# AlexandreRouma/qdsp

Hardware: AMD Instinct MI355X
Metric: Msamples/s complex IQ through 256-tap FIR+decimate chain, 1/2/4/8 GPU (higher is better)
Workload: dtype f32; 1 GPU; 256-tap complex FIR (real taps), synthetic IQ resident in HBM (BASELINE configs[1]); ntaps=256, decim=1, halo_samples=0, partition=single stream

## Files before the change

qdsp_amd/csrc/fft_fir.hip:

```cpp
#include "fft_fir.hip.h"
#ifndef QDSP_HIP_DIAG
#define QDSP_HIP_DIAG 0
#endif
#include "cfft.hip.h"
#include "cpk.hip.h"
#include "ldsdma.hip.h"

namespace qk {

typedef float f4v __attribute__((ext_vector_type(4)));

__host__ __device__ constexpr int pos1(int e) { return (e >> 1) + 136 * (e & 1); }

template <int DEC, bool ROT, bool REAL = false>
__global__ __launch_bounds__(kFftNT, (DEC == 1 || !ROT) ? 4 : 3) void fir_fft_kernel(const FftArgs a) {
    __shared__ __attribute__((aligned(16))) float2 lds[kFftLdsElems + 16 * 17];
    __shared__ double2 s_pb[2];
    float2* tbl = lds + kFftLdsElems;
    const int t_lane = threadIdx.x, t = t_lane;
    const int H = a.H;
    const int te_lane = (t & ~63) | ((t & 31) << 1) | ((t >> 5) & 1);
    const int te = te_lane;
    constexpr int NS = 16 / DEC;
    constexpr int NACT = 256 / DEC;

    if ((int)blockIdx.x == a.nwg) {
        if constexpr (REAL) {
            const float* inr = reinterpret_cast<const float*>(a.in);
            const float* hr = reinterpret_cast<const float*>(a.hist);
            float* hn = reinterpret_cast<float*>(a.hist_next);
            for (int i = t; i < H; i += kFftNT) {
                const long long g = a.count - H + i;
                hn[i] = g < 0 ? hr[g + H] : inr[g];
            }
            return;
        }
        for (int i = t; i < H; i += kFftNT) {
            const long long g = a.count - H + i;
            float2 v;
            if (g < 0) {
                v = a.hist_keep[g + H];
                if (ROT && a.hist_raw_next) a.hist_raw_next[i] = a.hist[g + H];
            } else {
                v = a.in[g];
                if (ROT) {
                    const double2 p = fx_phasor(a.phase_in0 + (unsigned long long)g * a.dphase);
                    const float gain = fmaf((float)(int)(g & 511), a.gm1, 1.0f);
                    if (a.hist_raw_next) a.hist_raw_next[i] = make_float2(v.x * gain, v.y * gain);
                    v = cmulc<false>(v, make_float2((float)p.x * gain, (float)p.y * gain));
                }
            }
            a.hist_next[i] = v;
        }
        return;
    }

    float2 ta[16], hf[16];
#pragma unroll
    for (int k = 0; k < 16; k++) {
        hf[k] = a.Hf[t * 16 + k];
        if (DEC == 1) ta[k] = a.TA[te * 16 + k];
    }
    const int e0 = ((t / NS) * 16 + (t % NS) * DEC) & 255;
    tbl[(t >> 4) * 17 + (t & 15)] = a.TB[t];

    float2 pl = make_float2(1.0f, 0.0f);
    if (ROT) {
        const double2 p = fx_phasor((unsigned long long)(DEC == 1 ? te : e0) * a.dphase);
        pl = make_float2((float)p.x, (float)p.y);
        if (t == 0) s_pb[0] = fx_phasor(a.phase0 + (unsigned long long)((long long)blockIdx.x * a.L - a.seg_shift) * a.dphase);
    }
    int seg_parity = 0;

    for (int b = blockIdx.x; b < a.nblocks; b += a.nwg) {
        int t_seg = t_lane;
        if constexpr (DEC == 1 ? (ROT || REAL) : !ROT) asm volatile("" : "+v"(t_seg));
        const int t = t_seg, hi = t >> 4, lo = t & 15;
        const int te = (t & ~63) | ((t & 31) << 1) | ((t >> 5) & 1), half = (t >> 5) & 1, pte = pos1(te);
        const float2* tb = tbl + lo * 17;
        const long long seg0 = (long long)(REAL ? 2 * b : b) * a.L - a.seg_shift;
        const long long segB = seg0 + a.L;
        const bool interior = seg0 >= 0 && (REAL ? segB : seg0) + kFftN <= a.count;
        float2 v[16];
        if constexpr (REAL) {
            const float* __restrict__ inr = reinterpret_cast<const float*>(a.in);
            const float* __restrict__ hr = reinterpret_cast<const float*>(a.hist);
            if (interior && a.vec) {
                const float2* __restrict__ pa = reinterpret_cast<const float2*>(inr + seg0 + (te & ~1)) + half * 8 * 128;
                const float2* __restrict__ pb = reinterpret_cast<const float2*>(inr + segB + (te & ~1)) + half * 8 * 128;
#pragma unroll
                for (int r = 0; r < 8; r++) {
                    const float2 qa = pa[r * 128], qb = pb[r * 128];
                    const auto sa = __builtin_amdgcn_permlane32_swap(__float_as_uint(qa.x), __float_as_uint(qa.y), false, false);
                    const auto sb = __builtin_amdgcn_permlane32_swap(__float_as_uint(qb.x), __float_as_uint(qb.y), false, false);
// ... 35 lines not shown
                const long long g = seg0 + n2 * 256 + te;
                float2 x = make_float2(0.0f, 0.0f);
                if (g < 0) { if (g + H >= 0) x = a.hist[g + H]; }
                else if (g < a.count) x = a.in[g];
                v[n2] = x;
            }
        }
        float2 q = make_float2(1.0f, 0.0f);
        if (ROT) {
            if (a.gm1 != 0.0f) {
                const int gb = (int)((seg0 + te) & 511);
                const float g0 = fmaf((float)gb, a.gm1, 1.0f), g1 = fmaf((float)(gb ^ 256), a.gm1, 1.0f);
                const bool nohist = seg0 >= 0;
#pragma unroll
                for (int n2 = 0; n2 < 16; n2++) {
                    const float gg = (n2 & 1) ? g1 : g0;
                    if (nohist || seg0 + n2 * 256 + te >= 0) v[n2] = make_float2(v[n2].x * gg, v[n2].y * gg);
                }
            }
        }
        auto make_q = [&]() {
            if (!ROT) return;
            const double2 pbv = s_pb[seg_parity];
            q = cmulc<false>(make_float2((float)pbv.x, (float)pbv.y), pl);
            if (t == 0) s_pb[seg_parity ^ 1] = dcmul(pbv, a.rot_step);
            seg_parity ^= 1;
        };
        auto rot_out = [&](int n2, float2 y) {
            if (!ROT) return y;
            return cmulc<false>(y, (n2 == 0) ? q : cmulc<false>(q, a.wtab[n2]));
        };
        fft16<false>(v);
        if constexpr (DEC > 1) {
            const float2* tap = a.TA + te * 16;
            asm volatile("" : "+v"(tap) : "v"(v[0].x));
#pragma unroll
            for (int k = 1; k < 16; k++) ta[k] = tap[k];
        }
        __syncthreads();
#pragma unroll
        for (int k = 0; k < 16; k++) lds[k * kFftRow1 + pte] = (k == 0) ? v[rev16(0)] : cmulc<false>(v[rev16(k)], ta[k]);
        __syncthreads();
#pragma unroll
        for (int j = 0; j < 16; j++) v[j] = lds[hi * kFftRow1 + pos1(j * 16 + lo)];
        fft16<false>(v);
        __syncthreads();
#pragma unroll
        for (int k = 0; k < 16; k++)
            lds[(hi * 16 + k) * kFftRow2 + lo] = (k == 0) ? v[rev16(0)] : cmulc<false>(v[rev16(k)], tb[k]);
        __syncthreads();
#pragma unroll
        for (int j = 0; j < 16; j++) v[j] = lds[t * kFftRow2 + j];
        fft16<false>(v);
        float2 y[16];
#pragma unroll
        for (int k = 0; k < 16; k++) y[k] = cmulc<false>(v[rev16(k)], hf[k]);
        fft16<true>(y);
        __syncthreads();
        if constexpr (DEC == 1) {
#pragma unroll
            for (int j = 0; j < 16; j++)
                lds[t * kFftRow2 + j] = (j == 0) ? y[rev16(0)] : cmulc<true>(y[rev16(j)], tb[j]);
            __syncthreads();
#pragma unroll
            for (int j = 0; j < 16; j++) v[j] = lds[(hi * 16 + j) * kFftRow2 + lo];
            fft16<true>(v);
            __syncthreads();
#pragma unroll
            for (int j = 0; j < 16; j++) lds[hi * kFftRow1 + pos1(j * 16 + lo)] = v[rev16(j)];
            __syncthreads();
// ... 73 lines not shown
                        o4[r * 128] = make_float4(__uint_as_float(sx[0]), __uint_as_float(sy[0]), __uint_as_float(sx[1]), __uint_as_float(sy[1]));
                }
            } else if (interior) {
#pragma unroll
                for (int n2 = 0; n2 < 16; n2++)
                    if (n2 * 256 + te >= a.ov) a.out[o0 + n2 * 256] = v[rev16(n2)];
            } else {
#pragma unroll
                for (int n2 = 0; n2 < 16; n2++) {
                    const long long n = o0 + n2 * 256;
                    if (n2 * 256 + te >= a.ov && n < a.nout) a.out[n] = v[rev16(n2)];
                }
            }
        } else {
#pragma unroll
            for (int s = 0; s < NS; s++) {
                const int n0 = s * DEC;
                lds[(hi * NS + s) * kFftRow2 + lo] = (n0 == 0) ? y[rev16(0)] : cmulc<true>(y[rev16(n0)], tb[n0]);
            }
            __syncthreads();
            if (t < NACT) {
#pragma unroll
                for (int j = 0; j < 16; j++) v[j] = lds[t * kFftRow2 + j];
                fft16<true>(v);
            }
            __syncthreads();
            if (t < NACT) {
                const int k0 = t / NS, s = t % NS;
#pragma unroll
                for (int j = 0; j < 16; j++) lds[(j * NS + s) * kFftRow2 + k0] = v[rev16(j)];
            }
            __syncthreads();
            if (t < NACT) {
                const float2* ta2 = a.TA + e0 * 16;
                asm volatile("" : "+v"(ta2) : "v"(v[0].x));
#pragma unroll
                for (int k = 0; k < 16; k++) {
                    const float2 e = lds[t * kFftRow2 + k];
                    v[k] = (k == 0) ? e : cmulc<true>(e, ta2[k]);
                }
                fft16<true>(v);
                make_q();
                const long long nb = ((long long)b * a.L - a.ov) / DEC;
                float2* __restrict__ seg_out = a.out + nb;
                const long long left = a.nout - nb;
                const int end_out = left < kFftN ? (int)left : kFftN;
#pragma unroll
                for (int n2 = 0; n2 < 16; n2++) {
                    const int i = n2 * 256 + e0;
                    if (i >= a.ov && i / DEC < end_out) seg_out[i / DEC] = rot_out(n2, v[rev16(n2)]);
                }
            }
        }
    }
}

#define QK_LDS_BARRIER() asm volatile("s_waitcnt lgkmcnt(0)\n\ts_barrier" ::: "memory")

__global__ __launch_bounds__(kFftNT, 4) void fir_fft_dma_kernel(const FftArgs a) {
    __shared__ __attribute__((aligned(16))) float2 lds[kFftLdsElems + 16 * 17];
    float2* tbl = lds + kFftLdsElems;
    const int t = threadIdx.x;
    const int hi = t >> 4, lo = t & 15;
    const int H = a.H;
    const int half = (t >> 4) & 1;
    const int te = (t & ~31) | ((t & 15) << 1) | half;

    if ((int)blockIdx.x == a.nwg) {
        for (int i = t; i < H; i += kFftNT) {
            const long long g = a.count - H + i;
            a.hist_next[i] = g < 0 ? a.hist_keep[g + H] : a.in[g];
        }
        return;
    }
    float2 ta[16], hf[16];
#pragma unroll
    for (int k = 0; k < 16; k++) {
        hf[k] = a.Hf[t * 16 + k];
        ta[k] = a.TA[te * 16 + k];
    }
    tbl[(t >> 4) * 17 + (t & 15)] = a.TB[t];
    const float2* tb = tbl + lo * 17;
    {
        float touch = 0.0f;
#pragma unroll
        for (int k = 0; k < 16; k++) touch += hf[k].x + hf[k].y + (k ? ta[k].x + ta[k].y : 0.0f);
        asm volatile("" ::"v"(touch));
    }
    __syncthreads();

    const int wcol = __builtin_amdgcn_readfirstlane(t & ~63);
    const unsigned lds_cols = __builtin_amdgcn_readfirstlane((unsigned)(uintptr_t)lds) + (unsigned)wcol * 8u;
    const unsigned voff = (unsigned)(t & 31) * 16u;
    auto seg_start = [&](int b) { return (long long)b * a.L - a.seg_shift; };
    auto is_interior = [&](int b) {
        const long long s0 = seg_start(b);
        return b < a.nblocks && s0 >= 0 && s0 + kFftN <= a.count;
    };
    auto request = [&](int b) {
        const float2* src = a.in + seg_start(b) + wcol;
        if ((t & 32) == 0) {
#pragma unroll
            for (int n2 = 0; n2 < 16; n2++) dma16_to_lds(src + n2 * 256, voff, lds_cols + (unsigned)(n2 * kFftRow1) * 8u);
        }
    };

    int b = blockIdx.x;
    bool landed_in_lds = false, eight_younger = false;
    if (b < a.nblocks && is_interior(b)) {
        request(b);
        landed_in_lds = true;
    }
    for (; b < a.nblocks; b += a.nwg) {
        const long long seg0 = seg_start(b);
        float2 v[16];
        if (landed_in_lds) {
            if (eight_younger) asm volatile("s_waitcnt vmcnt(8)" ::: "memory");
            else asm volatile("s_waitcnt vmcnt(0)" ::: "memory");
        } else {
            const int first_in = seg0 < 0 ? (int)-seg0 : 0;
            const int end_in = a.count - seg0 < kFftN ? (int)(a.count - seg0) : kFftN;
            const float2* __restrict__ seg_in = a.in + seg0;
            const float2* __restrict__ seg_hist = a.hist + (H - first_in);
            int tev = te;
            asm volatile("" : "+v"(tev));
#pragma unroll
            for (int n2 = 0; n2 < 16; n2++) {
                const int i = n2 * 256 + tev;
                float2 x = make_float2(0.0f, 0.0f);
                if (i < first_in) { if (i - first_in + H >= 0) x = seg_hist[i]; }
                else if (i < end_in) x = seg_in[i];
                lds[n2 * kFftRow1 + te] = x;
            }
        }
#pragma unroll
        for (int n2 = 0; n2 < 16; n2++) v[n2] = lds[n2 * kFftRow1 + te];
        fft16<false>(v);
#pragma unroll
        for (int k = 0; k < 16; k++) lds[k * kFftRow1 + te] = (k == 0) ? v[rev16(0)] : cmulc<false>(v[rev16(k)], ta[k]);
        QK_LDS_BARRIER();
#pragma unroll
        for (int j = 0; j < 16; j++) v[j] = lds[hi * kFftRow1 + j * 16 + lo];
        fft16<false>(v);
        QK_LDS_BARRIER();
#pragma unroll
        for (int k = 0; k < 16; k++)
            lds[(hi * 16 + k) * kFftRow2 + lo] = (k == 0) ? v[rev16(0)] : cmulc<false>(v[rev16(k)], tb[k]);
        QK_LDS_BARRIER();
#pragma unroll
        for (int j = 0; j < 16; j++) v[j] = lds[t * kFftRow2 + j];
        fft16<false>(v);
        float2 y[16];
#pragma unroll
        for (int k = 0; k < 16; k++) y[k] = cmulc<false>(v[rev16(k)], hf[k]);
        fft16<true>(y);
        QK_LDS_BARRIER();
#pragma unroll
        for (int j = 0; j < 16; j++)
            lds[t * kFftRow2 + j] = (j == 0) ? y[rev16(0)] : cmulc<true>(y[rev16(j)], tb[j]);
        QK_LDS_BARRIER();
#pragma unroll
        for (int j = 0; j < 16; j++) v[j] = lds[(hi * 16 + j) * kFftRow2 + lo];
        fft16<true>(v);
        QK_LDS_BARRIER();
#pragma unroll
        for (int j = 0; j < 16; j++) lds[hi * kFftRow1 + j * 16 + lo] = v[rev16(j)];
        QK_LDS_BARRIER();
        float2 e[16];
#pragma unroll
        for (int k = 0; k < 16; k++) e[k] = lds[k * kFftRow1 + te];
        const int nb = b + a.nwg;
        landed_in_lds = is_interior(nb);
        if (landed_in_lds) {
            asm volatile("s_waitcnt lgkmcnt(0)" ::: "memory");
            request(nb);
        }
#pragma unroll
        for (int k = 0; k < 16; k++) v[k] = (k == 0) ? e[k] : cmulc<true>(e[k], ta[k]);
        fft16<true>(v);
        eight_younger = false;
        if (seg0 >= 0 && seg0 + kFftN <= a.nout) {
            f4v* __restrict__ o4 = reinterpret_cast<f4v*>(a.out + seg0);
            int pair = (te >> 1) + half * 8 * 128;
            asm volatile("" : "+v"(pair));
#pragma unroll
            for (int r = 0; r < 8; r++) {
                const float2 lo_row = v[rev16(r)], hi_row = v[rev16(8 + r)];
                const auto sx = __builtin_amdgcn_permlane16_swap(__float_as_uint(lo_row.x), __float_as_uint(hi_row.x), false, false);
                const auto sy = __builtin_amdgcn_permlane16_swap(__float_as_uint(lo_row.y), __float_as_uint(hi_row.y), false, false);
                if ((half * 8 + r) * 256 + (te & ~1) >= a.ov)
                    o4[pair + r * 128] = (f4v){__uint_as_float(sx[0]), __uint_as_float(sy[0]), __uint_as_float(sx[1]), __uint_as_float(sy[1])};
            }
            eight_younger = true;
        } else {
            const int first_out = seg0 < 0 ? (int)-seg0 : 0;
            const int from = a.ov > first_out ? a.ov : first_out;
            const int end_out = a.nout - seg0 < kFftN ? (int)(a.nout - seg0) : kFftN;
            float2* __restrict__ seg_out = a.out + seg0;
            int tev = te;
            asm volatile("" : "+v"(tev));
#pragma unroll
            for (int n2 = 0; n2 < 16; n2++) {
                const int i = n2 * 256 + tev;
                if (i >= from && i < end_out) seg_out[i] = v[rev16(n2)];
            }
        }
    }
    asm volatile("s_waitcnt vmcnt(0)" ::: "memory");
}

template <bool CONJ, int ABL> __device__ __forceinline__ v2f abl_cmul(v2f a, v2f b) {
    if (ABL & 1) return a;
    return pk_cmul2<CONJ>(a, b);
}

template <bool STAMPS, int ABL = 0>
__global__ __launch_bounds__(kFftNT, 4) void fir_fft_dmapk_kernel(const FftArgs a) {
    __shared__ __attribute__((aligned(16))) v2f lds[kFftLdsElems + 16 * 17];
    v2f* tbl = lds + kFftLdsElems;
    const int t = threadIdx.x;
    const int hi = t >> 4, lo = t & 15;
    const int H = a.H;
    const int half = (t >> 4) & 1;
    const int te = (t & ~31) | ((t & 15) << 1) | half;

    if ((int)blockIdx.x == a.nwg) {
        for (int i = t; i < H; i += kFftNT) {
            const long long g = a.count - H + i;
            a.hist_next[i] = g < 0 ? a.hist_keep[g + H] : a.in[g];
        }
        return;
    }
    v2f ta[16], hf[16];
#pragma unroll
    for (int k = 0; k < 16; k++) {
        hf[k] = reinterpret_cast<const v2f*>(a.Hf)[t * 16 + k];
        ta[k] = reinterpret_cast<const v2f*>(a.TA)[te * 16 + k];
    }
    tbl[(t >> 4) * 17 + (t & 15)] = reinterpret_cast<const v2f*>(a.TB)[t];
    const v2f* tb = tbl + lo * 17;
    {
        float touch = 0.0f;
#pragma unroll
        for (int k = 0; k < 16; k++) touch += hf[k].x + hf[k].y + (k ? ta[k].x + ta[k].y : 0.0f);
        asm volatile("" ::"v"(touch));
    }
    __syncthreads();

    const int wcol = __builtin_amdgcn_readfirstlane(t & ~63);
    const unsigned lds_cols = __builtin_amdgcn_readfirstlane((unsigned)(uintptr_t)lds) + (unsigned)wcol * 8u;
    const unsigned voff = (unsigned)(t & 31) * 16u;
    auto seg_start = [&](int b) { return (long long)b * a.L - a.seg_shift; };
    auto is_interior = [&](int b) {
        const long long s0 = seg_start(b);
        return b < a.nblocks && s0 >= 0 && s0 + kFftN <= a.count;
    };
    auto request = [&](int b) {
        const float2* src = a.in + seg_start(b) + wcol;
        if ((t & 32) == 0 && !(ABL & 4)) {
            if (a.nt & 1) {
#pragma unroll
                for (int n2 = 0; n2 < 16; n2++) {
                    if (n2 == 0 || n2 == 15) dma16_to_lds(src + n2 * 256, voff, lds_cols + (unsigned)(n2 * kFftRow1) * 8u);
                    else dma16_to_lds_nt(src + n2 * 256, voff, lds_cols + (unsigned)(n2 * kFftRow1) * 8u);
                }
            } else {
#pragma unroll
                for (int n2 = 0; n2 < 16; n2++) dma16_to_lds(src + n2 * 256, voff, lds_cols + (unsigned)(n2 * kFftRow1) * 8u);
            }
        }
    };

    unsigned acc[16] = {0, 0, 0, 0, 0, 0, 0, 0, 0, 0, 0, 0, 0, 0, 0, 0};
    unsigned long long tick = 0;
    if constexpr (STAMPS) tick = __builtin_amdgcn_s_memtime();
#define QK_STAMP(i)                                                          \
    if constexpr (STAMPS) {                                                  \
        const unsigned long long now_ = __builtin_amdgcn_s_memtime();        \
        acc[i] += (unsigned)(now_ - tick);                                   \
        tick = now_;                                                         \
    }
    int b = blockIdx.x;
    bool landed_in_lds = false, eight_younger = false;
    if (b < a.nblocks && is_interior(b)) {
        request(b);
        landed_in_lds = true;
    }
    for (; b < a.nblocks; b += a.nwg) {
        const long long seg0 = seg_start(b);
        v2f v[16];
        QK_STAMP(15)
        if (landed_in_lds) {
            if (eight_younger) asm volatile("s_waitcnt vmcnt(8)" ::: "memory");
            else asm volatile("s_waitcnt vmcnt(0)" ::: "memory");
            QK_STAMP(0)
        } else {
            const int first_in = seg0 < 0 ? (int)-seg0 : 0;
            const int end_in = a.count - seg0 < kFftN ? (int)(a.count - seg0) : kFftN;
            const float2* __restrict__ seg_in = a.in + seg0;
            const float2* __restrict__ seg_hist = a.hist + (H - first_in);
            int tev = te;
            asm volatile("" : "+v"(tev));
#pragma unroll
            for (int n2 = 0; n2 < 16; n2++) {
                const int i = n2 * 256 + tev;
                float2 x = make_float2(0.0f, 0.0f);
                if (i < first_in) { if (i - first_in + H >= 0) x = seg_hist[i]; }
                else if (i < end_in) x = seg_in[i];
                lds[n2 * kFftRow1 + te] = mk2(x.x, x.y);
            }
        }
#pragma unroll
        for (int n2 = 0; n2 < 16; n2++) v[n2] = lds[n2 * kFftRow1 + te];
        if (!(ABL & 1)) pk_fft16<false>(v);
#pragma unroll
        for (int k = 0; k < 16; k++) lds[k * kFftRow1 + te] = (k == 0) ? v[rev16(0)] : abl_cmul<false, ABL>(v[rev16(k)], ta[k]);
        QK_STAMP(1)
        QK_LDS_BARRIER();
        QK_STAMP(2)
#pragma unroll
        for (int j = 0; j < 16; j++) v[j] = lds[hi * kFftRow1 + j * 16 + lo];
// ... 7 lines not shown
        QK_STAMP(5)
        QK_LDS_BARRIER();
        QK_STAMP(6)
#pragma unroll
        for (int j = 0; j < 16; j++) v[j] = lds[t * kFftRow2 + j];
        if (!(ABL & 1)) pk_fft16<false>(v);
        v2f y[16];
#pragma unroll
        for (int k = 0; k < 16; k++) y[k] = abl_cmul<false, ABL>(v[rev16(k)], hf[k]);
        if (!(ABL & 1)) pk_fft16<true>(y);
        QK_STAMP(7)
        QK_LDS_BARRIER();
        QK_STAMP(8)
#pragma unroll
        for (int j = 0; j < 16; j++)
            lds[t * kFftRow2 + j] = (j == 0) ? y[rev16(0)] : abl_cmul<true, ABL>(y[rev16(j)], tb[j]);
        QK_STAMP(9)
        QK_LDS_BARRIER();
        QK_STAMP(10)
#pragma unroll
        for (int j = 0; j < 16; j++) v[j] = lds[(hi * 16 + j) * kFftRow2 + lo];
        if (!(ABL & 1)) pk_fft16<true>(v);
        QK_STAMP(11)
        QK_LDS_BARRIER();
        QK_STAMP(12)
#pragma unroll
        for (int j = 0; j < 16; j++) lds[hi * kFftRow1 + j * 16 + lo] = v[rev16(j)];
        QK_STAMP(13)
        QK_LDS_BARRIER();
        QK_STAMP(14)
        v2f e[16];
#pragma unroll
        for (int k = 0; k < 16; k++) e[k] = lds[k * kFftRow1 + te];
        const int nb = b + a.nwg;
        landed_in_lds = is_interior(nb);
        if (landed_in_lds) {
            asm volatile("s_waitcnt lgkmcnt(0)" ::: "memory");
            request(nb);
        }
#pragma unroll
        for (int k = 0; k < 16; k++) v[k] = (k == 0) ? e[k] : abl_cmul<true, ABL>(e[k], ta[k]);
        if (!(ABL & 1)) pk_fft16<true>(v);
        eight_younger = false;
        if (seg0 >= 0 && seg0 + kFftN <= a.nout) {
            f4v* __restrict__ o4 = reinterpret_cast<f4v*>(a.out + seg0);
            int pair = (te >> 1) + half * 8 * 128;
            asm volatile("" : "+v"(pair));
            const bool nts = (a.nt & 2) != 0;
#pragma unroll
            for (int r = 0; r < 8; r++) {
                const v2f lo_row = v[rev16(r)], hi_row = v[rev16(8 + r)];
                const auto sx = __builtin_amdgcn_permlane16_swap(__float_as_uint(lo_row.x), __float_as_uint(hi_row.x), false, false);
                const auto sy = __builtin_amdgcn_permlane16_swap(__float_as_uint(lo_row.y), __float_as_uint(hi_row.y), false, false);
                if ((half * 8 + r) * 256 + (te & ~1) >= a.ov) {
                    const f4v o = {__uint_as_float(sx[0]), __uint_as_float(sy[0]), __uint_as_float(sx[1]), __uint_as_float(sy[1])};
                    if (ABL & 2) { if (o.x == 1.2345e30f) o4[pair + r * 128] = o; }
                    else if (nts) __builtin_nontemporal_store(o, o4 + pair + r * 128);
                    else o4[pair + r * 128] = o;
                }
            }
            eight_younger = true;
        } else {
            const int first_out = seg0 < 0 ? (int)-seg0 : 0;
            const int from = a.ov > first_out ? a.ov : first_out;
            const int end_out = a.nout - seg0 < kFftN ? (int)(a.nout - seg0) : kFftN;
            v2f* __restrict__ seg_out = reinterpret_cast<v2f*>(a.out) + seg0;
            int tev = te;
            asm volatile("" : "+v"(tev));
#pragma unroll
            for (int n2 = 0; n2 < 16; n2++) {
                const int i = n2 * 256 + tev;
                if (i >= from && i < end_out) seg_out[i] = v[rev16(n2)];
            }
        }
    }
    asm volatile("s_waitcnt vmcnt(0)" ::: "memory");
    if constexpr (STAMPS) {
        if (t == 0) {
#pragma unroll
            for (int q = 0; q < 16; q++) a.stamps[(long long)blockIdx.x * 16 + q] = acc[q];
        }
    }
#undef QK_STAMP
}

template <int DEC, bool ROT>
__global__ __launch_bounds__(kFftNT, 2) void fir_fft_dec_kernel(const FftArgs a) {
    __shared__ __attribute__((aligned(16))) float2 lds[2 * kFftLdsElems + 16 * 17];
    float2* stage = lds + kFftLdsElems;
    float2* tbl = lds + 2 * kFftLdsElems;
    const int t = threadIdx.x;
    const int hi = t >> 4, lo = t & 15;
    const int H = a.H;
    constexpr int NS = 16 / DEC;
    constexpr int NACT = 256 / DEC;

    if ((int)blockIdx.x == a.nwg) {
        for (int i = t; i < H; i += kFftNT) {
            const long long g = a.count - H + i;
            float2 v;
            if (g < 0) {
                v = a.hist_keep[g + H];
                if (ROT && a.hist_raw_next) a.hist_raw_next[i] = a.hist[g + H];
            } else {
                v = a.in[g];
                if (ROT) {
                    const double2 p = fx_phasor(a.phase_in0 + (unsigned long long)g * a.dphase);
                    const float gain = fmaf((float)(int)(g & 511), a.gm1, 1.0f);
                    if (a.hist_raw_next) a.hist_raw_next[i] = make_float2(v.x * gain, v.y * gain);
                    v = cmulc<false>(v, make_float2((float)p.x * gain, (float)p.y * gain));
                }
            }
            a.hist_next[i] = v;
        }
        return;
    }

    float2 ta[16], hf[16];
    const int wbb = t / NACT, wr = t % NACT;
    const int e0 = (wr / NS) * 16 + (wr % NS) * DEC;
#pragma unroll
    for (int k = 0; k < 16; k++) {
        hf[k] = a.Hf[t * 16 + k];
        ta[k] = a.TA[t * 16 + k];
    }
    tbl[(t >> 4) * 17 + (t & 15)] = a.TB[t];
    const float2* tb = tbl + lo * 17;

    float2 pl = make_float2(1.0f, 0.0f);
    if (ROT) {
        const double2 p = fx_phasor((unsigned long long)e0 * a.dphase);
        pl = make_float2((float)p.x, (float)p.y);
    }

    auto load_segment = [&](int b, float2 (&v)[16]) {
        const long long seg0 = (long long)b * a.L - a.seg_shift;
        if (b < a.nblocks && seg0 >= 0 && seg0 + kFftN <= a.count) {
            const float2* __restrict__ p = a.in + seg0 + t;
#pragma unroll
            for (int n2 = 0; n2 < 16; n2++) v[n2] = p[n2 * 256];
        } else {
#pragma unroll
            for (int n2 = 0; n2 < 16; n2++) {
                const long long g = seg0 + n2 * 256 + t;
                float2 x = make_float2(0.0f, 0.0f);
                if (b < a.nblocks) {
                    if (g < 0) { if (g + H >= 0) x = a.hist[g + H]; }
                    else if (g < a.count) x = a.in[g];
                }
                v[n2] = x;
            }
        }
    };

    const int ngroups = (a.nblocks + DEC - 1) / DEC;
    double2 pbg = make_double2(1.0, 0.0);
    if (ROT) pbg = fx_phasor(a.phase0 + (unsigned long long)((long long)((int)blockIdx.x * DEC + wbb) * a.L - a.seg_shift) * a.dphase);
// ... 46 lines not shown
            for (int r = 0; r < NS; r++) {
                gsum[r] = y[r];
#pragma unroll
                for (int k = r + NS; k < 16; k += NS) gsum[r] = cadd(gsum[r], y[k]);
            }
            if constexpr (NS == 4) fft4<true>(gsum[0], gsum[1], gsum[2], gsum[3]);
            if constexpr (NS == 2) {
                const float2 e = gsum[0], o = gsum[1];
                gsum[0] = cadd(e, o);
                gsum[1] = csub(e, o);
            }
#pragma unroll
            for (int s = 0; s < NS; s++) {
                const int n0 = s * DEC;
                stage[(bb * NACT + hi * NS + s) * kFftRow2 + lo] = (n0 == 0) ? gsum[0] : cmulc<true>(gsum[s], tb[n0]);
            }
            if (bb + 1 < DEC) {
#pragma unroll
                for (int n2 = 0; n2 < 16; n2++) v[n2] = vn[n2];
            }
        }
        __syncthreads();
#pragma unroll
        for (int j = 0; j < 16; j++) v[j] = stage[t * kFftRow2 + j];
        fft16<true>(v);
        {
            const int ubb = t / NACT, ur = t % NACT;
            const int k0 = ur / NS, s = ur % NS;
#pragma unroll
            for (int j = 0; j < 16; j++) lds[(ubb * NACT + j * NS + s) * kFftRow2 + k0] = v[rev16(j)];
        }
        __syncthreads();
        {
            const float2* ta2 = a.TA + e0 * 16;
            asm volatile("" : "+v"(ta2) : "v"(v[0].x));
#pragma unroll
            for (int k = 0; k < 16; k++) {
                const float2 e = lds[t * kFftRow2 + k];
                v[k] = (k == 0) ? e : cmulc<true>(e, ta2[k]);
            }
        }
        fft16<true>(v);
        const int b = b0 + wbb;
        const long long nb = ((long long)b * a.L - a.ov) / DEC;
#pragma unroll
        for (int n2 = 0; n2 < 16; n2++) {
            const int i = n2 * 256 + e0;
            const long long n = nb + i / DEC;
            float2 y = v[rev16(n2)];
            if (ROT) y = cmulc<false>(y, (n2 == 0) ? q : cmulc<false>(q, a.wtab[n2]));
            if (b < a.nblocks && i >= a.ov && n < a.nout) a.out[n] = y;
        }
    }
}

int launch_fir_fft(const FftArgs& a, int grid, hipStream_t stream) {
#define QK_FFT(dec, rot) hipLaunchKernelGGL((fir_fft_dec_kernel<dec, rot>), dim3(grid), dim3(kFftNT), 0, stream, a)
    const bool r = a.rot != 0;
    switch (a.dec) {
        case 1:
#if QDSP_HIP_DIAG
            if (a.dma == 2 && a.abl == 1) hipLaunchKernelGGL((fir_fft_dmapk_kernel<false, 1>), dim3(grid), dim3(kFftNT), 0, stream, a);
            else if (a.dma == 2 && a.abl == 2) hipLaunchKernelGGL((fir_fft_dmapk_kernel<false, 2>), dim3(grid), dim3(kFftNT), 0, stream, a);
            else if (a.dma == 2 && a.abl == 4) hipLaunchKernelGGL((fir_fft_dmapk_kernel<false, 4>), dim3(grid), dim3(kFftNT), 0, stream, a);
            else if (a.dma == 2 && a.abl == 6) hipLaunchKernelGGL((fir_fft_dmapk_kernel<false, 6>), dim3(grid), dim3(kFftNT), 0, stream, a);
            else if (a.dma == 2 && a.abl == 7) hipLaunchKernelGGL((fir_fft_dmapk_kernel<false, 7>), dim3(grid), dim3(kFftNT), 0, stream, a);
            else if (a.dma == 2 && a.stamps) hipLaunchKernelGGL(fir_fft_dmapk_kernel<true>, dim3(grid), dim3(kFftNT), 0, stream, a);
            else
#endif
            if (a.dma == 2) hipLaunchKernelGGL(fir_fft_dmapk_kernel<false>, dim3(grid), dim3(kFftNT), 0, stream, a);
            else if (a.dma) hipLaunchKernelGGL(fir_fft_dma_kernel, dim3(grid), dim3(kFftNT), 0, stream, a);
            else if (a.real2) hipLaunchKernelGGL((fir_fft_kernel<1, false, true>), dim3(grid), dim3(kFftNT), 0, stream, a);
// ... 21 lines not shown
```

qdsp_amd/csrc/fft_fir.hip.h:

```cpp
#pragma once
#include <hip/hip_runtime.h>
#include "kconst.h"

namespace qk {

constexpr int kFftNT = 256;
constexpr int kFftRow1 = 272;
constexpr int kFftRow2 = 17;
constexpr int kFftLdsElems = 16 * kFftRow1;

struct FftArgs {
    const float2* in;
    float2* out;
    const float2* hist;
    float2* hist_raw_next;
    const float2* hist_keep;
    float2* hist_next;
    const float2* Hf;
    const float2* TA;
    const float2* TB;
    long long count;
    long long nout;
    int H;
    int dec;
    int decm;
    unsigned decm_inv;
    int strided;
    int rot;
    int ov;
    int seg_shift;
    int L;
    int nblocks;
    int nwg;
    int vec;
    int grouped;
    int m_shift;
    int abl;
    unsigned* stamps;
    int nt;
    int dma;
    int real2;
    unsigned long long phase_in0;
    unsigned long long phase0;
    unsigned long long dphase;
    double2 rot_step;
    float2 wtab[16];
    float gm1;
};

constexpr int kFft1kN = 1024;
constexpr int kFft1kPitch = 84;
int launch_fir_fft1k(const FftArgs& a, hipStream_t stream);

int launch_fir_fft(const FftArgs& a, int grid, hipStream_t stream);

}
```

qdsp_amd/csrc/knobs.h:

```cpp
#pragma once
#include <atomic>

namespace qk {

#define QDSP_HIP_KNOBS(X) \
    X(ANY_SMALL_CALL_TILES) \
    X(CHAN_ABL) \
    X(CHAN_MAX_WG) X(CHAN_NO_ST4) X(DECIM_SETTING) X(FFT1K_MAX_COUNT) X(FFT_ABL) X(FFT_DMA) \
    X(FFT_MIN_TAPS_DECIM) X(FFT_MIN_TAPS_REAL) \
    X(FFT_MIN_TAPS_SMALL) X(FFT_NT) X(FFT_PRUNE2_MAX_COUNT) X(FFT_WG_PER_CU) X(FIR_LAT_MAX_WORK) X(FIR_MODE) X(FIR_PICK) X(FORCE_ANY) \
    X(LEVEL_ROW_TILES) \
    X(MF_BATCH_MIN_WORK) X(MF_DEPTH) X(MF_MIN_COUNT) X(MF_MIN_DECIM) \
    X(MF_TASK_MAX) X(NO_CHAN_BATCH) X(NO_DECIM_TABLE) X(NO_FFT1K) X(NO_FFT1K_REAL) X(NO_FIR_LAT) X(NO_FIR_TABLE) X(NO_LM) \
    X(NO_LM_SMALL_CALL_RULE) X(NO_MF) X(NO_MF_BATCH) X(NO_PFB) X(NO_RM) X(NO_RM_EXT) X(NO_SPLIT_UPLOAD) \
    X(NO_WIN) X(NT) X(PFB_MIN_COUNT) X(PFB_WG_PER_CU) X(R) X(RM_MIN_COUNT) X(RM_MIN_INTERP) \
    X(RM_WAVES_PER_SIMD) X(WIN_MAX_TAPS) X(WIN_R) 
enum Knob {
#define X(n) K_##n,
    QDSP_HIP_KNOBS(X)
#undef X
    K_COUNT
};

struct Knobs {
    int val[K_COUNT];
    unsigned char set[K_COUNT];
    unsigned long long fft_stamps;
};

const Knobs* knobs_snapshot();
void knobs_reload();

inline int knob(Knob k, int dflt) {
    const Knobs* s = knobs_snapshot();
    return s->set[k] ? s->val[k] : dflt;
}

}
```

qdsp_amd/csrc/qdsp_hip.hip:

```cpp
#include "engine.hip.h"

namespace qh {

Engine* as_engine(void* h, Kind k) {
    Engine* e = static_cast<Engine*>(h);
    if (!e || e->magic != kMagic || e->kind != k) return nullptr;
    return e;
}

long double turns_of(float re, float im) {
    const long double two_pi = 6.283185307179586476925286766559005768L;
    long double t = atan2l((long double)im, (long double)re) / two_pi;
    t -= floorl(t);
    return t;
}
unsigned long long fx_of_turns(long double t) {
    t -= floorl(t);
    long double s = ldexpl(t, 64);
    if (s >= 18446744073709551615.0L) return 0ULL;
    return (unsigned long long)s;
}
void unit_of_fx(unsigned long long ph, long double mult, double* c, double* s) {
    const long double two_pi = 6.283185307179586476925286766559005768L;
    long double t = ldexpl((long double)ph, -64) * mult;
// ... 534 lines not shown
}

void reversed_taps(const Engine* e, std::vector<long double>& gr, std::vector<long double>& gi) {
    const long double two_pi = 6.283185307179586476925286766559005768L;
    const int N = e->ntaps;
    for (int j = 0; j < N; j++) {
        const long double h = (long double)e->taps_host[N - 1 - j];
        long double c = 1.0L, sn = 0.0L;
        if (e->rotate) {
            const long double tt = ldexpl((long double)e->dphase, -64) * (long double)(N - 1 - j);
            c = cosl(two_pi * (tt - floorl(tt)));
            sn = sinl(two_pi * (tt - floorl(tt)));
        }
        gr[j] = h * c;
        gi[j] = h * sn;
    }
}

int fft_prepare(Engine* e) {
    const unsigned long long key_dphase = e->rotate ? e->dphase : 0;
    if (e->fft_ntaps == e->ntaps && e->fft_tw_ready && e->fft_dphase == key_dphase) return 0;
    constexpr int F = qk::kFftN;
    const long double two_pi = 6.283185307179586476925286766559005768L;
    std::vector<long double> cs, sn;
    if (!e->fft_tw_ready) {
        cs.resize(F);
        sn.resize(F);
        for (int i = 0; i < F; i++) {
            cs[i] = cosl(two_pi * (long double)i / F);
            sn[i] = sinl(two_pi * (long double)i / F);
        }
    }
    const int N = e->ntaps;
    std::vector<float2> Hp(F), TA(256 * 16), TB(16 * 16);
    std::vector<long double> gr(N), gi(N);
    reversed_taps(e, gr, gi);
    std::vector<double> sre, sim;
    host_spectrum(gr, gi, F, sre, sim);
    for (int k = 0; k < F; k++) {
        const int k0 = k & 15, k1 = (k >> 4) & 15, k2 = k >> 8;
        Hp[(k0 * 16 + k1) * 16 + k2] = make_float2((float)(sre[k] / F), (float)(sim[k] / F));
    }
    if (!e->fft_tw_ready) {
        for (int t = 0; t < 256; t++)
            for (int k = 0; k < 16; k++) TA[t * 16 + k] = make_float2((float)cs[(t * k) % F], (float)(-sn[(t * k) % F]));
        for (int lo = 0; lo < 16; lo++)
            for (int k = 0; k < 16; k++) TB[lo * 16 + k] = make_float2((float)cs[(16 * lo * k) % F], (float)(-sn[(16 * lo * k) % F]));
        if (!e->d_fft_H) HIPCHK(hipMalloc(&e->d_fft_H, sizeof(float2) * F));
        if (!e->d_fft_TA) HIPCHK(hipMalloc(&e->d_fft_TA, sizeof(float2) * 256 * 16));
        if (!e->d_fft_TB) HIPCHK(hipMalloc(&e->d_fft_TB, sizeof(float2) * 16 * 16));
        HIPCHK(hipMemcpy(e->d_fft_TA, TA.data(), sizeof(float2) * TA.size(), hipMemcpyHostToDevice));
        HIPCHK(hipMemcpy(e->d_fft_TB, TB.data(), sizeof(float2) * TB.size(), hipMemcpyHostToDevice));
        e->fft_tw_ready = true;
    }
    HIPCHK(hipDeviceSynchronize());
    HIPCHK(hipMemcpy(e->d_fft_H, Hp.data(), sizeof(float2) * F, hipMemcpyHostToDevice));
    e->fft_ntaps = N;
    e->fft_dphase = key_dphase;
    return 0;
}

int fft1k_prepare(Engine* e) {
    const unsigned long long key_dphase = e->rotate ? e->dphase : 0;
    if (e->f1k_ntaps == e->ntaps && e->f1k_tw_ready && e->f1k_dphase == key_dphase) return 0;
    constexpr int F = qk::kFft1kN;
    const long double two_pi = 6.283185307179586476925286766559005768L;
    std::vector<long double> cs, sn;
    if (!e->f1k_tw_ready) {
        cs.resize(F);
        sn.resize(F);
        for (int i = 0; i < F; i++) {
            cs[i] = cosl(two_pi * (long double)i / F);
            sn[i] = sinl(two_pi * (long double)i / F);
        }
    }
    const int N = e->ntaps;
    std::vector<long double> gr(N), gi(N);
    reversed_taps(e, gr, gi);
    std::vector<float2> Hp(F), T(64 * 16 + 4 * 16);
    std::vector<double> sre, sim;
    host_spectrum(gr, gi, F, sre, sim);
    for (int k = 0; k < F; k++) {
        const double re = sre[k], im = sim[k];
        const int ka = k & 15, kb1 = (k >> 4) & 15, kb0 = k >> 8;
        Hp[(4 * (kb1 & 3) + kb0) * 64 + ((ka << 2) | (kb1 >> 2))] = make_float2((float)(re / F), (float)(im / F));
    }
    if (!e->f1k_tw_ready) {
        for (int l = 0; l < 64; l++)
            for (int k = 0; k < 16; k++) T[k * 64 + l] = make_float2((float)cs[(l * k) % F], (float)(-sn[(l * k) % F]));
// ... 251 lines not shown
        unit_of_fx(a.phase0 - (unsigned long long)(8 * (a.Q - 1) + 1) * a.dphase, 1.0L, &a.pb_base.x, &a.pb_base.y);
        for (int k = 0; k < 12; k++) unit_of_fx_c(e->dphase, 8.0L * (long double)a.Lo * (long double)(1 << k), &a.seg_pow[k].x, &a.seg_pow[k].y);
        for (int b1 = 0; b1 < 8; b1++) {
            double c, sn;
            unit_of_fx_c(e->dphase, (long double)(512 * b1), &c, &sn);
            a.wtab[b1] = make_float2((float)c, (float)sn);
        }
    }
    rc = qk::launch_pfb_dec(a, s);
    if (rc) return rc;
    e->raw_valid = e->rotate && e->H > 0;
    e->last.name = a.real ? (a.PH == 2 ? "pfb_dec4_real_kernel" : "pfb_dec8_real_kernel") : a.PH == 2 ? "pfb_dec4_kernel" : "pfb_dec8_kernel";
    e->last.grid = nwg + 1;
    e->last.block = qk::kPfbNT * a.PH;
    e->last.lds = (int)((qk::kPfbTableElems + (a.PH - 1) * qk::kPfbG1Elems + wpw * 64 * qk::kPfbRow + (a.PH - 1) * wpw * 64 * 9) * sizeof(float2));
    return 0;
}

int launch_fft(Engine* e, const void* d_in, int64_t count, int64_t nout, void* d_out, hipStream_t s) {
    int rc = fft_prepare(e);
    if (rc) return rc;
    qk::FftArgs a;
    memset(&a, 0, sizeof(a));
    a.in = static_cast<const float2*>(d_in);
    a.out = static_cast<float2*>(d_out);
    a.hist = reinterpret_cast<const float2*>(e->d_hist[e->cur]);
    a.hist_keep = a.hist;
    a.hist_next = reinterpret_cast<float2*>(e->d_hist[e->cur ^ 1]);
    rc = raw_history(e, s, &a.hist, &a.hist_raw_next);
    if (rc) return rc;
    a.Hf = e->d_fft_H;
    a.TA = e->d_fft_TA;
    a.TB = e->d_fft_TB;
    a.count = count;
    a.nout = nout;
    a.H = e->H;
    a.dec = fft_dec(desc_of(e));
    if (a.dec == 2 && e->ch == 2) {
        const int lim = qk::knob(qk::K_FFT_PRUNE2_MAX_COUNT, -1);
        if (count >= (lim >= 0 ? (int64_t)lim : (int64_t)(e->rotate ? 1 << 25 : 1 << 24))) a.dec = 1;
    }
    a.rot = e->rotate ? 1 : 0;
    a.decm = 1;
    if (a.dec == 1 && e->kind != KIND_FIR) {
        a.decm = e->M;
        a.decm_inv = (e->M >= 2 && (unsigned long long)(e->M + 4096) * (unsigned long long)e->M < (1ULL << 32)) ? (unsigned)((1ULL << 32) / (unsigned)e->M) + 1u : 0u;
        a.strided = 1;
        a.ov = (e->ntaps - 1 + 1) & ~1;
        a.seg_shift = a.ov + 2;
        a.L = qk::kFftN - a.ov;
        a.nblocks = (int)((count + 2 + a.L - 1) / a.L);
        a.vec = (((uintptr_t)d_in) & 15) == 0;
    } else if (a.dec == 1) {
        a.ov = (e->ntaps - 1 + 1) & ~1;
        a.vec = ((((uintptr_t)d_in) | ((uintptr_t)d_out)) & 15) == 0;
        a.seg_shift = a.ov;
        a.L = qk::kFftN - a.ov;
        a.nblocks = (int)((count + a.L - 1) / a.L);
    } else {
        a.ov = ((e->ntaps - 1 + a.dec - 1) / a.dec) * a.dec;
        a.seg_shift = a.ov + 1;
        a.L = qk::kFftN - a.ov;
        const int per_block = a.L / a.dec;
        a.nblocks = (int)((nout + per_block - 1) / per_block);
    }
    if (e->ch == 1) {
        a.real2 = 1;
        a.vec = ((((uintptr_t)d_in) | ((uintptr_t)d_out)) & 7) == 0;
        a.nblocks = (a.nblocks + 1) / 2;
    }
    a.nt = qk::knob(qk::K_FFT_NT, 0);
    a.abl = qk::knob(qk::K_FFT_ABL, 0);
    a.stamps = reinterpret_cast<unsigned*>(qk::knobs_snapshot()->fft_stamps);
    a.dma = (a.dec == 1 && !a.strided && !a.rot && e->ch == 2 && a.vec && a.ov <= 2048) ? qk::knob(qk::K_FFT_DMA, 1) : 0;
    const bool grouped = a.dec >= 4 && (a.nblocks + a.dec - 1) / a.dec >= 1024;
    a.grouped = grouped ? 1 : 0;
    const int per_cu = qk::knob(qk::K_FFT_WG_PER_CU, grouped ? 4 : 16);
    const int units = grouped ? (a.nblocks + a.dec - 1) / a.dec : a.nblocks;
    int nwg = 256 * per_cu;
    if (nwg > units) nwg = units;
    a.nwg = nwg;
    if (a.rot) {
        a.phase_in0 = e->phase;
        a.phase0 = e->phase - (unsigned long long)(e->ntaps - 1) * e->dphase;
        a.dphase = e->dphase;
        a.gm1 = e->volk_gain ? e->gm1 : 0.0f;
        const long double step_mult = (long double)nwg * (long double)a.L * (long double)(grouped ? a.dec : 1);
        if (!e->rot_step_ok || e->rot_step_dphase != e->dphase || e->rot_step_mult != step_mult) {
            unit_of_fx_c(e->dphase, step_mult, &e->rot_step_val.x, &e->rot_step_val.y);
            e->rot_step_dphase = e->dphase;
            e->rot_step_mult = step_mult;
            e->rot_step_ok = true;
        }
        a.rot_step = e->rot_step_val;
        if (!e->wtab4k_ok || e->wtab4k_dphase != e->dphase) {
            for (int n2 = 0; n2 < 16; n2++) {
                double c, sn;
                unit_of_fx_c(e->dphase, (long double)(256 * n2), &c, &sn);
                e->wtab4k[n2] = make_float2((float)c, (float)sn);
            }
            e->wtab4k_dphase = e->dphase;
            e->wtab4k_ok = true;
        }
        memcpy(a.wtab, e->wtab4k, sizeof(a.wtab));
    }
    rc = qk::launch_fir_fft(a, nwg + 1, s);
    if (rc) return rc;
    e->raw_valid = e->rotate && e->H > 0;
    e->last.name = a.dma == 2 ? "fir_fft_dmapk_kernel" : a.dma ? "fir_fft_dma_kernel" : "fir_fft_kernel";
    e->last.grid = nwg + 1;
    e->last.block = qk::kFftNT;
    e->last.lds = (int)(((grouped ? 2 : 1) * qk::kFftLdsElems + 16 * 17) * sizeof(float2));
    return 0;
// ... 761 lines not shown
```

Measured before the change: 309,400 Msamples/s.

## Taper FFT-FIR DMA block schedule and transpose twiddle tables for coalesced loads

Adds transposed copies of the filter spectrum and twiddle tables so per-thread table loads read consecutive addresses across lanes, selected by a new knob that is on by default. In the DMA kernels, the grid-strided block loop becomes a tapered schedule: a set of long-running workgroups handles the first several rounds, and the remaining blocks are split into shrinking tiers spread over extra workgroups to reduce tail imbalance. It also adds realtime and hardware-register stamps in the diagnostic path. In exchange it doubles table memory, and the DMA path now uses a different workgroups-per-CU default (4 instead of 16) when computing slots, which changes how many workgroups are resident.

Measured after the change: 317,200 Msamples/s (median of 6 runs). 2.5% higher.

```diff
diff --git a/qdsp_amd/csrc/fft_fir.hip b/qdsp_amd/csrc/fft_fir.hip
--- a/qdsp_amd/csrc/fft_fir.hip
+++ b/qdsp_amd/csrc/fft_fir.hip
@@ -11,6 +11,15 @@
 typedef float f4v __attribute__((ext_vector_type(4)));
 
 __host__ __device__ constexpr int pos1(int e) { return (e >> 1) + 136 * (e & 1); }
+
+struct FftTbl {
+    const float2 *hf, *ta;
+    int ks;
+    unsigned ls;
+};
+__device__ __forceinline__ FftTbl fft_tbl(const FftArgs& a) {
+    return a.tbl ? FftTbl{a.HfT, a.TAT, 256, 1u} : FftTbl{a.Hf, a.TA, 1, 16u};
+}
 
 template <int DEC, bool ROT, bool REAL = false>
 __global__ __launch_bounds__(kFftNT, (DEC == 1 || !ROT) ? 4 : 3) void fir_fft_kernel(const FftArgs a) {
@@ -55,11 +64,12 @@
         return;
     }
 
+    const FftTbl T = fft_tbl(a);
     float2 ta[16], hf[16];
 #pragma unroll
     for (int k = 0; k < 16; k++) {
-        hf[k] = a.Hf[t * 16 + k];
-        if (DEC == 1) ta[k] = a.TA[te * 16 + k];
+        hf[k] = (T.hf + k * T.ks)[(unsigned)t * T.ls];
+        if (DEC == 1) ta[k] = (T.ta + k * T.ks)[(unsigned)te * T.ls];
     }
     const int e0 = ((t / NS) * 16 + (t % NS) * DEC) & 255;
     tbl[(t >> 4) * 17 + (t & 15)] = a.TB[t];
@@ -161,10 +171,11 @@
         };
         fft16<false>(v);
         if constexpr (DEC > 1) {
-            const float2* tap = a.TA + te * 16;
-            asm volatile("" : "+v"(tap) : "v"(v[0].x));
-#pragma unroll
-            for (int k = 1; k < 16; k++) ta[k] = tap[k];
+            unsigned tap = (unsigned)te * T.ls;
+            int ks = T.ks;
+            asm volatile("" : "+v"(tap), "+s"(ks) : "v"(v[0].x));
+#pragma unroll
+            for (int k = 1; k < 16; k++) ta[k] = (T.ta + k * ks)[tap];
         }
         __syncthreads();
 #pragma unroll
@@ -304,12 +315,13 @@
             }
             __syncthreads();
             if (t < NACT) {
-                const float2* ta2 = a.TA + e0 * 16;
-                asm volatile("" : "+v"(ta2) : "v"(v[0].x));
+                unsigned ta2 = (unsigned)e0 * T.ls;
+                int ks = T.ks;
+                asm volatile("" : "+v"(ta2), "+s"(ks) : "v"(v[0].x));
 #pragma unroll
                 for (int k = 0; k < 16; k++) {
                     const float2 e = lds[t * kFftRow2 + k];
-                    v[k] = (k == 0) ? e : cmulc<true>(e, ta2[k]);
+                    v[k] = (k == 0) ? e : cmulc<true>(e, (T.ta + k * ks)[ta2]);
                 }
                 fft16<true>(v);
                 make_q();
@@ -328,6 +340,28 @@
 }
 
 #define QK_LDS_BARRIER() asm volatile("s_waitcnt lgkmcnt(0)\n\ts_barrier" ::: "memory")
+
+__device__ __forceinline__ void fft_run_of(const FftArgs& a, int w, int& b, int& step, int& left) {
+    if (w < a.n_long) {
+        b = w;
+        step = a.n_long;
+        left = (a.nblocks - w + a.n_long - 1) / a.n_long;
+        if (left > a.rounds) left = a.rounds;
+        return;
+    }
+    int seg = a.rounds * a.n_long, wg = a.n_long, rem = a.nblocks - seg, len = 1;
+    while (rem > 0) {
+        int cnt;
+        len = fft_taper_tier(rem, a.n_long, cnt);
+        if (w < wg + cnt) break;
+        wg += cnt;
+        seg += cnt * len;
+        rem -= cnt * len;
+    }
+    b = seg + (w - wg) * len;
+    step = 1;
+    left = a.nblocks - b < len ? a.nblocks - b : len;
+}
 
 __global__ __launch_bounds__(kFftNT, 4) void fir_fft_dma_kernel(const FftArgs a) {
     __shared__ __attribute__((aligned(16))) float2 lds[kFftLdsElems + 16 * 17];
@@ -345,22 +379,6 @@
         }
         return;
     }
-    float2 ta[16], hf[16];
-#pragma unroll
-    for (int k = 0; k < 16; k++) {
-        hf[k] = a.Hf[t * 16 + k];
-        ta[k] = a.TA[te * 16 + k];
-    }
-    tbl[(t >> 4) * 17 + (t & 15)] = a.TB[t];
-    const float2* tb = tbl + lo * 17;
-    {
-        float touch = 0.0f;
-#pragma unroll
-        for (int k = 0; k < 16; k++) touch += hf[k].x + hf[k].y + (k ? ta[k].x + ta[k].y : 0.0f);
-        asm volatile("" ::"v"(touch));
-    }
-    __syncthreads();
-
     const int wcol = __builtin_amdgcn_readfirstlane(t & ~63);
     const unsigned lds_cols = __builtin_amdgcn_readfirstlane((unsigned)(uintptr_t)lds) + (unsigned)wcol * 8u;
     const unsigned voff = (unsigned)(t & 31) * 16u;
@@ -377,13 +395,30 @@
         }
     };
 
-    int b = blockIdx.x;
+    const FftTbl T = fft_tbl(a);
+    float2 ta[16], hf[16];
+#pragma unroll
+    for (int k = 0; k < 16; k++) {
+        hf[k] = (T.hf + k * T.ks)[(unsigned)t * T.ls];
+        ta[k] = (T.ta + k * T.ks)[(unsigned)te * T.ls];
+    }
+    tbl[(t >> 4) * 17 + (t & 15)] = a.TB[t];
+    const float2* tb = tbl + lo * 17;
+    {
+        float touch = 0.0f;
+#pragma unroll
+        for (int k = 0; k < 16; k++) touch += hf[k].x + hf[k].y + (k ? ta[k].x + ta[k].y : 0.0f);
+        asm volatile("" ::"v"(touch));
+    }
+    __syncthreads();
+    int b, step, left;
+    fft_run_of(a, blockIdx.x, b, step, left);
     bool landed_in_lds = false, eight_younger = false;
-    if (b < a.nblocks && is_interior(b)) {
+    if (left > 0 && is_interior(b)) {
         request(b);
         landed_in_lds = true;
     }
-    for (; b < a.nblocks; b += a.nwg) {
+    for (; left > 0; left--, b += step) {
         const long long seg0 = seg_start(b);
         float2 v[16];
         if (landed_in_lds) {
@@ -441,8 +476,8 @@
         float2 e[16];
 #pragma unroll
         for (int k = 0; k < 16; k++) e[k] = lds[k * kFftRow1 + te];
-        const int nb = b + a.nwg;
-        landed_in_lds = is_interior(nb);
+        const int nb = b + step;
+        landed_in_lds = left > 1 && is_interior(nb);
         if (landed_in_lds) {
             asm volatile("s_waitcnt lgkmcnt(0)" ::: "memory");
             request(nb);
@@ -490,6 +525,8 @@
 __global__ __launch_bounds__(kFftNT, 4) void fir_fft_dmapk_kernel(const FftArgs a) {
     __shared__ __attribute__((aligned(16))) v2f lds[kFftLdsElems + 16 * 17];
     v2f* tbl = lds + kFftLdsElems;
+    unsigned long long rt_first = 0;
+    if constexpr (STAMPS) rt_first = __builtin_amdgcn_s_memrealtime();
     const int t = threadIdx.x;
     const int hi = t >> 4, lo = t & 15;
     const int H = a.H;
@@ -503,22 +540,6 @@
         }
         return;
     }
-    v2f ta[16], hf[16];
-#pragma unroll
-    for (int k = 0; k < 16; k++) {
-        hf[k] = reinterpret_cast<const v2f*>(a.Hf)[t * 16 + k];
-        ta[k] = reinterpret_cast<const v2f*>(a.TA)[te * 16 + k];
-    }
-    tbl[(t >> 4) * 17 + (t & 15)] = reinterpret_cast<const v2f*>(a.TB)[t];
-    const v2f* tb = tbl + lo * 17;
-    {
-        float touch = 0.0f;
-#pragma unroll
-        for (int k = 0; k < 16; k++) touch += hf[k].x + hf[k].y + (k ? ta[k].x + ta[k].y : 0.0f);
-        asm volatile("" ::"v"(touch));
-    }
-    __syncthreads();
-
     const int wcol = __builtin_amdgcn_readfirstlane(t & ~63);
     const unsigned lds_cols = __builtin_amdgcn_readfirstlane((unsigned)(uintptr_t)lds) + (unsigned)wcol * 8u;
     const unsigned voff = (unsigned)(t & 31) * 16u;
@@ -543,22 +564,43 @@
         }
     };
 
+    const FftTbl T = fft_tbl(a);
+    v2f ta[16], hf[16];
+#pragma unroll
+    for (int k = 0; k < 16; k++) {
+        hf[k] = reinterpret_cast<const v2f*>(T.hf + k * T.ks)[(unsigned)t * T.ls];
+        ta[k] = reinterpret_cast<const v2f*>(T.ta + k * T.ks)[(unsigned)te * T.ls];
+    }
+    tbl[(t >> 4) * 17 + (t & 15)] = reinterpret_cast<const v2f*>(a.TB)[t];
+    const v2f* tb = tbl + lo * 17;
+    {
+        float touch = 0.0f;
+#pragma unroll
+        for (int k = 0; k < 16; k++) touch += hf[k].x + hf[k].y + (k ? ta[k].x + ta[k].y : 0.0f);
+        asm volatile("" ::"v"(touch));
+    }
+    __syncthreads();
+
     unsigned acc[16] = {0, 0, 0, 0, 0, 0, 0, 0, 0, 0, 0, 0, 0, 0, 0, 0};
-    unsigned long long tick = 0;
-    if constexpr (STAMPS) tick = __builtin_amdgcn_s_memtime();
+    unsigned long long tick = 0, rt_loop = 0;
+    if constexpr (STAMPS) {
+        tick = __builtin_amdgcn_s_memtime();
+        rt_loop = __builtin_amdgcn_s_memrealtime();
+    }
 #define QK_STAMP(i)                                                          \
     if constexpr (STAMPS) {                                                  \
         const unsigned long long now_ = __builtin_amdgcn_s_memtime();        \
         acc[i] += (unsigned)(now_ - tick);                                   \
         tick = now_;                                                         \
     }
-    int b = blockIdx.x;
+    int b, step, left;
+    fft_run_of(a, blockIdx.x, b, step, left);
     bool landed_in_lds = false, eight_younger = false;
-    if (b < a.nblocks && is_interior(b)) {
+    if (left > 0 && is_interior(b)) {
         request(b);
         landed_in_lds = true;
     }
-    for (; b < a.nblocks; b += a.nwg) {
+    for (; left > 0; left--, b += step) {
         const long long seg0 = seg_start(b);
         v2f v[16];
         QK_STAMP(15)
@@ -632,8 +674,8 @@
         v2f e[16];
 #pragma unroll
         for (int k = 0; k < 16; k++) e[k] = lds[k * kFftRow1 + te];
-        const int nb = b + a.nwg;
-        landed_in_lds = is_interior(nb);
+        const int nb = b + step;
+        landed_in_lds = left > 1 && is_interior(nb);
         if (landed_in_lds) {
             asm volatile("s_waitcnt lgkmcnt(0)" ::: "memory");
             request(nb);
@@ -677,8 +719,15 @@
     asm volatile("s_waitcnt vmcnt(0)" ::: "memory");
     if constexpr (STAMPS) {
         if (t == 0) {
-#pragma unroll
-            for (int q = 0; q < 16; q++) a.stamps[(long long)blockIdx.x * 16 + q] = acc[q];
+            unsigned* st = a.stamps + (long long)blockIdx.x * kFftStampWords;
+#pragma unroll
+            for (int q = 0; q < 16; q++) st[q] = acc[q];
+            const unsigned long long rt_last = __builtin_amdgcn_s_memrealtime();
+            st[16] = (unsigned)rt_first; st[17] = (unsigned)(rt_first >> 32);
+            st[18] = (unsigned)rt_loop;  st[19] = (unsigned)(rt_loop >> 32);
+            st[20] = (unsigned)rt_last;  st[21] = (unsigned)(rt_last >> 32);
+            st[22] = __builtin_amdgcn_s_getreg((31 << 11) | 4);
+            st[23] = __builtin_amdgcn_s_getreg((3 << 11) | 20);
         }
     }
 #undef QK_STAMP
@@ -716,13 +765,14 @@
         return;
     }
 
+    const FftTbl T = fft_tbl(a);
     float2 ta[16], hf[16];
     const int wbb = t / NACT, wr = t % NACT;
     const int e0 = (wr / NS) * 16 + (wr % NS) * DEC;
 #pragma unroll
     for (int k = 0; k < 16; k++) {
-        hf[k] = a.Hf[t * 16 + k];
-        ta[k] = a.TA[t * 16 + k];
+        hf[k] = (T.hf + k * T.ks)[(unsigned)t * T.ls];
+        ta[k] = (T.ta + k * T.ks)[(unsigned)t * T.ls];
     }
     tbl[(t >> 4) * 17 + (t & 15)] = a.TB[t];
     const float2* tb = tbl + lo * 17;
@@ -835,12 +885,13 @@
         }
         __syncthreads();
         {
-            const float2* ta2 = a.TA + e0 * 16;
-            asm volatile("" : "+v"(ta2) : "v"(v[0].x));
+            unsigned ta2 = (unsigned)e0 * T.ls;
+            int ks = T.ks;
+            asm volatile("" : "+v"(ta2), "+s"(ks) : "v"(v[0].x));
 #pragma unroll
             for (int k = 0; k < 16; k++) {
                 const float2 e = lds[t * kFftRow2 + k];
-                v[k] = (k == 0) ? e : cmulc<true>(e, ta2[k]);
+                v[k] = (k == 0) ? e : cmulc<true>(e, (T.ta + k * ks)[ta2]);
             }
         }
         fft16<true>(v);
diff --git a/qdsp_amd/csrc/fft_fir.hip.h b/qdsp_amd/csrc/fft_fir.hip.h
--- a/qdsp_amd/csrc/fft_fir.hip.h
+++ b/qdsp_amd/csrc/fft_fir.hip.h
@@ -9,6 +9,8 @@
 constexpr int kFftRow2 = 17;
 constexpr int kFftLdsElems = 16 * kFftRow1;
 
+constexpr int kFftStampWords = 24;
+
 struct FftArgs {
     const float2* in;
     float2* out;
@@ -19,6 +21,9 @@
     const float2* Hf;
     const float2* TA;
     const float2* TB;
+    const float2* HfT;
+    const float2* TAT;
+    int tbl;
     long long count;
     long long nout;
     int H;
@@ -32,6 +37,7 @@
     int L;
     int nblocks;
     int nwg;
+    int n_long, rounds;
     int vec;
     int grouped;
     int m_shift;
@@ -48,6 +54,28 @@
     float gm1;
 };
 
+inline int fft_taper_rounds(int nblocks, int slots) {
+    if (nblocks <= slots) return 1;
+    return nblocks / slots - nblocks / (4 * slots);
+}
+__host__ __device__ inline int fft_taper_tier(int rem, int slots, int& cnt) {
+    const int len = (rem + 2 * slots - 1) / (2 * slots);
+    cnt = (rem + len - 1) / len;
+    if (cnt > slots) cnt = slots;
+    return len;
+}
+inline int fft_taper_short_count(int nblocks, int slots, int rounds) {
+    const int n_long = nblocks < slots ? nblocks : slots;
+    int rem = nblocks - rounds * n_long, total = 0;
+    while (rem > 0) {
+        int cnt;
+        const int len = fft_taper_tier(rem, slots, cnt);
+        total += cnt;
+        rem -= cnt * len;
+    }
+    return total;
+}
+
 constexpr int kFft1kN = 1024;
 constexpr int kFft1kPitch = 84;
 int launch_fir_fft1k(const FftArgs& a, hipStream_t stream);
diff --git a/qdsp_amd/csrc/knobs.h b/qdsp_amd/csrc/knobs.h
--- a/qdsp_amd/csrc/knobs.h
+++ b/qdsp_amd/csrc/knobs.h
@@ -8,7 +8,7 @@
     X(CHAN_ABL) \
     X(CHAN_MAX_WG) X(CHAN_NO_ST4) X(DECIM_SETTING) X(FFT1K_MAX_COUNT) X(FFT_ABL) X(FFT_DMA) \
     X(FFT_MIN_TAPS_DECIM) X(FFT_MIN_TAPS_REAL) \
-    X(FFT_MIN_TAPS_SMALL) X(FFT_NT) X(FFT_PRUNE2_MAX_COUNT) X(FFT_WG_PER_CU) X(FIR_LAT_MAX_WORK) X(FIR_MODE) X(FIR_PICK) X(FORCE_ANY) \
+    X(FFT_MIN_TAPS_SMALL) X(FFT_NT) X(FFT_PRUNE2_MAX_COUNT) X(FFT_TBL) X(FFT_WG_PER_CU) X(FIR_LAT_MAX_WORK) X(FIR_MODE) X(FIR_PICK) X(FORCE_ANY) \
     X(LEVEL_ROW_TILES) \
     X(MF_BATCH_MIN_WORK) X(MF_DEPTH) X(MF_MIN_COUNT) X(MF_MIN_DECIM) \
     X(MF_TASK_MAX) X(NO_CHAN_BATCH) X(NO_DECIM_TABLE) X(NO_FFT1K) X(NO_FFT1K_REAL) X(NO_FIR_LAT) X(NO_FIR_TABLE) X(NO_LM) \
diff --git a/qdsp_amd/csrc/qdsp_hip.hip b/qdsp_amd/csrc/qdsp_hip.hip
--- a/qdsp_amd/csrc/qdsp_hip.hip
+++ b/qdsp_amd/csrc/qdsp_hip.hip
@@ -590,29 +590,29 @@
         }
     }
     const int N = e->ntaps;
-    std::vector<float2> Hp(F), TA(256 * 16), TB(16 * 16);
+    std::vector<float2> Hp(2 * F), TA(2 * 256 * 16), TB(16 * 16);
     std::vector<long double> gr(N), gi(N);
     reversed_taps(e, gr, gi);
     std::vector<double> sre, sim;
     host_spectrum(gr, gi, F, sre, sim);
     for (int k = 0; k < F; k++) {
         const int k0 = k & 15, k1 = (k >> 4) & 15, k2 = k >> 8;
-        Hp[(k0 * 16 + k1) * 16 + k2] = make_float2((float)(sre[k] / F), (float)(sim[k] / F));
+        Hp[(k0 * 16 + k1) * 16 + k2] = Hp[F + k2 * 256 + (k0 * 16 + k1)] = make_float2((float)(sre[k] / F), (float)(sim[k] / F));
     }
     if (!e->fft_tw_ready) {
         for (int t = 0; t < 256; t++)
-            for (int k = 0; k < 16; k++) TA[t * 16 + k] = make_float2((float)cs[(t * k) % F], (float)(-sn[(t * k) % F]));
+            for (int k = 0; k < 16; k++) TA[t * 16 + k] = TA[F + k * 256 + t] = make_float2((float)cs[(t * k) % F], (float)(-sn[(t * k) % F]));
         for (int lo = 0; lo < 16; lo++)
             for (int k = 0; k < 16; k++) TB[lo * 16 + k] = make_float2((float)cs[(16 * lo * k) % F], (float)(-sn[(16 * lo * k) % F]));
-        if (!e->d_fft_H) HIPCHK(hipMalloc(&e->d_fft_H, sizeof(float2) * F));
-        if (!e->d_fft_TA) HIPCHK(hipMalloc(&e->d_fft_TA, sizeof(float2) * 256 * 16));
+        if (!e->d_fft_H) HIPCHK(hipMalloc(&e->d_fft_H, sizeof(float2) * 2 * F));
+        if (!e->d_fft_TA) HIPCHK(hipMalloc(&e->d_fft_TA, sizeof(float2) * 2 * 256 * 16));
         if (!e->d_fft_TB) HIPCHK(hipMalloc(&e->d_fft_TB, sizeof(float2) * 16 * 16));
         HIPCHK(hipMemcpy(e->d_fft_TA, TA.data(), sizeof(float2) * TA.size(), hipMemcpyHostToDevice));
         HIPCHK(hipMemcpy(e->d_fft_TB, TB.data(), sizeof(float2) * TB.size(), hipMemcpyHostToDevice));
         e->fft_tw_ready = true;
     }
     HIPCHK(hipDeviceSynchronize());
-    HIPCHK(hipMemcpy(e->d_fft_H, Hp.data(), sizeof(float2) * F, hipMemcpyHostToDevice));
+    HIPCHK(hipMemcpy(e->d_fft_H, Hp.data(), sizeof(float2) * Hp.size(), hipMemcpyHostToDevice));
     e->fft_ntaps = N;
     e->fft_dphase = key_dphase;
     return 0;
@@ -930,6 +930,9 @@
     a.Hf = e->d_fft_H;
     a.TA = e->d_fft_TA;
     a.TB = e->d_fft_TB;
+    a.HfT = e->d_fft_H + qk::kFftN;
+    a.TAT = e->d_fft_TA + qk::kFftN;
+    a.tbl = qk::knob(qk::K_FFT_TBL, 1) ? 1 : 0;
     a.count = count;
     a.nout = nout;
     a.H = e->H;
@@ -977,6 +980,14 @@
     const int units = grouped ? (a.nblocks + a.dec - 1) / a.dec : a.nblocks;
     int nwg = 256 * per_cu;
     if (nwg > units) nwg = units;
+    a.n_long = nwg;
+    a.rounds = (units + nwg - 1) / (nwg > 0 ? nwg : 1);
+    if (a.dma) {
+        const int slots = 256 * qk::knob(qk::K_FFT_WG_PER_CU, 4);
+        a.n_long = a.nblocks < slots ? a.nblocks : slots;
+        a.rounds = qk::fft_taper_rounds(a.nblocks, slots);
+        nwg = a.n_long + qk::fft_taper_short_count(a.nblocks, slots, a.rounds);
+    }
     a.nwg = nwg;
     if (a.rot) {
         a.phase_in0 = e->phase;
```
